# indygreg/python-zstandard

Measured on AMD Instinct MI355X. Metric: GB/s uncompressed throughput, batch decompress of 128 KiB level-3 frames (the decompress half of BASELINE.json's metric; the compress half on the same inputs is this line's 'compress' object), higher is better.
Workload: dtype u8

## Files before the change

python-zstandard_amd/csrc/zhip_decode_kernel.hpp:

```cpp
#pragma once
#include "zhip_device.hpp"
#include "zhip_format.hpp"
#include "zhip_xxh64.hpp"

#if defined(ZHIP_EMU) && defined(ZD_TRACE)
#include <stdio.h>
extern "C" { extern long zd_trace_pos; extern long zd_cur_frame; extern long zd_stat[16]; }
#define ZD_STAT(i, v) do { if (zh_lane() == 0) zd_stat[i] += (v); } while (0)
#define ZD_TRR(lo, n, what, a1, a2) do { if (zh_lane() == 0 && zd_trace_pos + 40 >= (long)(lo) && zd_trace_pos < (long)(lo) + (long)(n) + 40) fprintf(stderr, "[trace] f%ld range [%ld,+%ld) %s %ld %ld\n", zd_cur_frame, (long)(lo), (long)(n), what, (long)(a1), (long)(a2)); } while (0)
#define ZD_TR(pos, what, a1, a2, a3) do { if ((long)(pos) == zd_trace_pos) fprintf(stderr, "[trace] f%ld pos=%ld %s lane=%u %ld %ld %ld\n", zd_cur_frame, (long)(pos), what, zh_lane(), (long)(a1), (long)(a2), (long)(a3)); } while (0)
#else
#define ZD_TR(pos, what, a1, a2, a3) do { } while (0)
#define ZD_TRR(lo, n, what, a1, a2) do { } while (0)
#define ZD_STAT(i, v) do { } while (0)
#endif
#define ZD_STAGE_BYTES 512
#define ZD_ASM_BYTES 4096
#define ZD_COOP_LEN 32

ZH_CONST uint32_t zc_llBase[36] = {0,1,2,3,4,5,6,7,8,9,10,11,12,13,14,15,16,18,20,22,24,28,32,40,48,64,128,256,512,
                                   1024,2048,4096,8192,16384,32768,65536};
ZH_CONST uint8_t zc_llBits[36] = {0,0,0,0,0,0,0,0,0,0,0,0,0,0,0,0,1,1,1,1,2,2,3,3,4,6,7,8,9,10,11,12,13,14,15,16};
ZH_CONST uint32_t zc_mlBase[53] = {3,4,5,6,7,8,9,10,11,12,13,14,15,16,17,18,19,20,21,22,23,24,25,26,27,28,29,30,31,32,
                                   33,34,35,37,39,41,43,47,51,59,67,83,99,131,259,515,1027,2051,4099,8195,16387,32771,65539};
// ... 417 lines not shown
    }
    zh_sync();
    return (int)log;
}

ZH_DEVFN bool zd_huf_stream(const uint16_t* huf, uint32_t log, const uint8_t* src, uint32_t srcSize, uint8_t* out, uint32_t count)
{
    ZdPBits b;
    if (!zd_pb_init(b, src, srcSize)) return false;
    uint32_t i = 0;
    zd_pb_norm(b);
    while (i + 4 <= count) {
        uint32_t e0 = huf[zd_pb_peek(b, log)]; b.used += e0 >> 8;
        uint32_t e1 = huf[zd_pb_peek(b, log)]; b.used += e1 >> 8;
        uint32_t e2 = huf[zd_pb_peek(b, log)]; b.used += e2 >> 8;
        uint32_t e3 = huf[zd_pb_peek(b, log)]; b.used += e3 >> 8;
        if (b.used > 64) return false;
        zh_st32(out + i, (e0 & 255) | ((e1 & 255) << 8) | ((e2 & 255) << 16) | ((e3 & 255) << 24));
        i += 4;
        zd_pb_norm(b);
    }
    while (i < count) {
        uint32_t e = huf[zd_pb_peek(b, log)]; b.used += e >> 8;
        if (b.used > 64) return false;
        out[i++] = (uint8_t)e;
    }
    zd_pb_norm(b);
    return zd_pb_done(b);
}

struct ZdLitDefer { uint16_t* table; uint32_t maxLog; uint32_t taken, log, four, streamBytes; const uint8_t* streams;
                    const uint16_t* prevTable; uint32_t prevLog;
                    uint32_t shared, shareOK;
                    const ZpPre* pre; };
ZH_DEVFN int zd_literals(ZdLDS& L, ZdState& st, const uint8_t* src, uint32_t srcSize, uint8_t* lit, uint32_t blockMax, ZdProf& P,
                         ZdLitDefer* defer = nullptr)
{
    const uint32_t lane = zh_lane();
    if (srcSize < 1) return -ZE_CORRUPTION;
    uint32_t b0 = src[0], type = b0 & 3, fmt = (b0 >> 2) & 3;
    uint32_t hdr, regen, csize = 0, four = 0;
    st.litRLE = 0;
    if (type < 2) {
        if (fmt == 1) { if (srcSize < 2) return -ZE_CORRUPTION; hdr = 2; regen = zh_ld16(src) >> 4; }
        else if (fmt == 3) { if (srcSize < 3) return -ZE_CORRUPTION; hdr = 3; regen = zh_ld24(src) >> 4; }
        else { hdr = 1; regen = b0 >> 3; }
        if (regen > blockMax) return -ZE_CORRUPTION;
        st.litSize = regen;
        if (type == 0) {
            if (hdr + regen > srcSize) return -ZE_CORRUPTION;
            st.litPtr = src + hdr;
            return (int)(hdr + regen);
        }
        if (hdr + 1 > srcSize) return -ZE_CORRUPTION;
        st.litRLE = 1; st.rleByte = src[hdr]; st.litPtr = lit;
        return (int)(hdr + 1);
    }
    if (srcSize < 5) return -ZE_CORRUPTION;
    uint32_t v = zh_ld32(src);
    if (fmt < 2) { hdr = 3; four = fmt; regen = (v >> 4) & 0x3FF; csize = (v >> 14) & 0x3FF; }
    else if (fmt == 2) { hdr = 4; four = 1; regen = (v >> 4) & 0x3FFF; csize = v >> 18; }
    else { hdr = 5; four = 1; regen = (v >> 4) & 0x3FFFF; csize = (v >> 22) + ((uint32_t)src[4] << 10); }
    if (regen > blockMax || regen > ZF_BLOCK_MAX) return -ZE_CORRUPTION;
    if (!four && regen == 0) return -ZE_CORRUPTION;
    if (four && regen < 6) return -ZE_CORRUPTION;
    if (hdr + csize > srcSize) return -ZE_CORRUPTION;
    const uint8_t* p = src + hdr; uint32_t left = csize;
    if (type == 3) {
        if (st.hufCount == 0) return -ZE_DICT_CORRUPTED;
    } else {
        uint32_t cnt = 0, lg = 0;
        int r = zd_read_huf_weights(L, p, left, &cnt, &lg, defer ? defer->pre : nullptr, hdr);
        if (r < 0) return -ZE_CORRUPTION;
        p += r; left -= (uint32_t)r; st.hufCount = cnt;
    }
    if (type == 3 && defer && defer->prevTable) {
        const int lgp = (int)defer->prevLog;
        if (four) {
            if (left < 10) return -ZE_CORRUPTION;
            if (3 * ((regen + 3) / 4) > regen) return -ZE_CORRUPTION;
        }
        if (defer->shareOK) defer->shared = 1;
        else {
            const uint64_t* t8 = (const uint64_t*)defer->prevTable; uint64_t* g8 = (uint64_t*)defer->table;
            for (uint32_t i = lane; i < (1u << lgp) / 4 + ((1u << lgp) < 4 ? 1u : 0u); i += 64) g8[i] = t8[i];
        }
        defer->taken = 1; defer->log = (uint32_t)lgp; defer->four = four; defer->streamBytes = left; defer->streams = p;
        ZD_T(P, ZP_HUFTAB);
        st.litPtr = lit; st.litSize = regen;
        return (int)(hdr + csize);
    }
    int lg = zd_build_huf(L, st.hufCount);
    if (lg < 0) return -ZE_CORRUPTION;
    if (defer && (uint32_t)lg <= defer->maxLog) {
        if (four) {
// ... 594 lines not shown
```

python-zstandard_amd/csrc/zhip_decode_pipeline.hpp:

```cpp
#pragma once
#include "zhip_decode_kernel.hpp"

ZH_DEV void zp_pack_fse(ZdLDS& L, uint32_t* T, uint32_t llLog, uint32_t ofLog, uint32_t mlLog)
{
    const uint32_t lane = zh_lane();
    for (uint32_t u = lane; u < ZP_FSE_CELLS / 2; u += 64) {
        const uint32_t lg = u < 256 ? llLog : u < 512 ? mlLog : ofLog;
        const uint32_t local = (2 * u) & (u < 512 ? 511u : 255u);
        uint32_t pair = 0;
        for (uint32_t k = 0; k < 2; k++) {
            uint32_t cell = 0;
            if (local + k < (1u << lg)) {
                const uint32_t e = L.fse[2 * u + k];
                cell = ((e >> 19) << 10) | (((e & 1023) + (1u << lg)) >> ((e >> 10) & 15));
            }
            pair |= cell << (16 * k);
        }
        T[u] = pair;
    }
}

struct ZpHdr { uint32_t pos, blockMax, hasChecksum, skippable; uint64_t fcs; };
ZH_DEV int zp_frame_header(const ZhipPipeArgs& a, const uint8_t* src, uint32_t srcSize, ZpHdr& h)
{
    const uint32_t mg = a.magicless ? 0u : 4u;
    h.skippable = 0;
    if (srcSize < mg + 1) return ZE_SRC_SIZE_WRONG;
    if (mg && (zh_ld32(src) & 0xFFFFFFF0u) == ZF_MAGIC_SKIPPABLE) {
        if (srcSize < 8 || (uint64_t)zh_ld32(src + 4) + 8 > srcSize) return ZE_SRC_SIZE_WRONG;
        h.skippable = 1; h.pos = 0; h.blockMax = 0; h.hasChecksum = 0; h.fcs = 0;
        return 0;
    }
    if (mg && zh_ld32(src) != ZF_MAGIC) return ZE_PREFIX_UNKNOWN;
    const uint32_t fhd = src[mg];
    const uint32_t dictCode = fhd & 3, single = (fhd >> 5) & 1, fcsCode = fhd >> 6;
    h.hasChecksum = (fhd >> 2) & 1;
    const uint32_t dictBytes = dictCode == 3 ? 4 : dictCode;
    const uint32_t fcsBytes = fcsCode == 0 ? single : (1u << fcsCode);
    const uint32_t hs = mg + 1 + (single ? 0 : 1) + dictBytes + fcsBytes;
    if (fhd & 8) return ZE_FRAMEPARAM_UNSUPPORTED;
    if (srcSize < hs) return ZE_SRC_SIZE_WRONG;
    uint32_t pos = mg + 1;
    uint64_t windowSize = 0;
    if (!single) {
        const uint32_t wd = src[pos++], wl = 10 + (wd >> 3);
        if (wl > 31) return ZE_WINDOW_TOO_LARGE;
        windowSize = 1ull << wl; windowSize += (windowSize >> 3) * (wd & 7);
    }
    {   const uint32_t dictID = dictCode == 0 ? 0u : dictCode == 1 ? src[pos] : dictCode == 2 ? zh_ld16(src + pos) : zh_ld32(src + pos);
        pos += dictBytes;
        if (dictID && dictID != a.dictID) return ZE_DICT_WRONG; }
    uint64_t fcs = ~0ull;
    if (fcsCode == 0) { if (single) fcs = src[pos]; }
    else if (fcsCode == 1) fcs = (uint64_t)zh_ld16(src + pos) + 256;
    else if (fcsCode == 2) fcs = zh_ld32(src + pos);
    else fcs = zh_ld64(src + pos);
    pos += fcsBytes;
    if (single) windowSize = fcs;
    if (windowSize > a.maxWindowSize) return ZE_WINDOW_TOO_LARGE;
    h.blockMax = windowSize < ZF_BLOCK_MAX ? (uint32_t)windowSize : ZF_BLOCK_MAX;
    h.fcs = fcs; h.pos = pos;
    return 0;
}

ZH_DEVFN int zp_block_tables(const ZhipPipeArgs& a, ZdLDS& L, ZdState& st, ZdLitDefer& df, const uint8_t* src, uint32_t pos, uint32_t bs,
                             uint32_t blockMax, uint32_t t, ZdMeta& m, ZdProf& P, bool share, bool dictInLds)
{
    const uint32_t lane = zh_lane();
    uint8_t* lit;
    {
        uint32_t need16 = 0;
        if (bs >= 5 && (src[pos] & 3u) >= 2u) {
            const uint32_t v = zh_ld32(src + pos), fmt = (v >> 2) & 3u;
            const uint32_t regen = fmt < 2 ? (v >> 4) & 0x3FFu : fmt == 2 ? (v >> 4) & 0x3FFFu : (v >> 4) & 0x3FFFFu;
            if (regen <= ZF_BLOCK_MAX) need16 = (regen + 256u + 15u) >> 4;
        }
        uint32_t lb = 0;
        if (need16) {
            lb = zh_first(zh_atomic_add(a.counters + 8, lane == 0 ? need16 : 0u));
            if ((uint64_t)lb + need16 > a.arenaBudget16) {
                if (zh_opaque(lane) == 0) zh_atomic_add(a.counters + 8, 0u - need16);
                return ZP_RC_FALLBACK;
            }
        }
        const uint32_t lpos = need16 ? a.arenaBudget16 - lb - need16 : 0u;
        lit = a.litArena + (size_t)lpos * 16;
        if (zh_opaque(lane) == 0) a.bases[2 * (size_t)t + 1] = lpos;
    }
    st.litPtr = lit; st.litSize = 0; st.litRLE = 0; st.rleByte = 0;
    const ZhipDictEntropy* const de = a.dictEntropy;
    const int r = zd_literals(L, st, src + pos, bs, lit, blockMax, P, &df);
    if (r < 0) return -r;
    m.litSize = st.litSize;
    if (df.taken) { m.litMode = 3u | (df.log << 8) | (df.four << 16) | (df.shared ? ZP_LIT_SHARED : 0u); m.litOff = (uint32_t)(df.streams - src); m.produced = df.streamBytes; }
    else if (st.litRLE) { m.litMode = 2; m.litOff = st.rleByte; }
    else if (st.litPtr == lit) { m.litMode = 1; m.litOff = 0; }
    else { m.litMode = 0; m.litOff = (uint32_t)(st.litPtr - src); }
    const uint8_t* sp = src + pos + (uint32_t)r; const uint8_t* const send = src + pos + bs;
    if (sp >= send) return ZE_SRC_SIZE_WRONG;
    uint32_t nbSeq = *sp++;
    if (nbSeq > 127) {
        if (nbSeq == 255) { if (sp + 2 > send) return ZE_SRC_SIZE_WRONG; nbSeq = zh_ld16(sp) + 0x7F00; sp += 2; }
        else { if (sp >= send) return ZE_SRC_SIZE_WRONG; nbSeq = ((nbSeq - 128) << 8) + *sp++; }
    }
    m.nbSeq = nbSeq;
    if (nbSeq == 0) { if (sp != send) return ZE_CORRUPTION; }
    else {
        if (nbSeq > ZP_SEQ_CAP - 16) return ZE_CORRUPTION;
        if (sp >= send) return ZE_SRC_SIZE_WRONG;
        const uint32_t modes = *sp++;
        if (modes & 3) return ZE_CORRUPTION;
        const bool allShared = share && de && (modes >> 2) == 0x3F;
        if (allShared) {
            st.llLog = de->llLog; st.ofLog = de->ofLog; st.mlLog = de->mlLog;
            if (sp >= send) return ZE_CORRUPTION;
        } else {
            if (de && !dictInLds) {
                zh_sync();
                const uint32_t* T = a.dictTables->fse;
                if ((modes >> 6) == 3) { for (uint32_t k = lane; k < (1u << de->llLog); k += 64) L.fse[ZD_FSE_LL + k] = T[ZD_FSE_LL + k]; st.llLog = de->llLog; }
                if (((modes >> 4) & 3) == 3) { for (uint32_t k = lane; k < (1u << de->ofLog); k += 64) L.fse[ZD_FSE_OF + k] = T[ZD_FSE_OF + k]; st.ofLog = de->ofLog; }
                if (((modes >> 2) & 3) == 3) { for (uint32_t k = lane; k < (1u << de->mlLog); k += 64) L.fse[ZD_FSE_ML + k] = T[ZD_FSE_ML + k]; st.mlLog = de->mlLog; }
                zh_sync();
            }
            const uint32_t hn = (uint32_t)(send - sp) < 256u ? (uint32_t)(send - sp) : 256u;
            uint8_t* const stg = (uint8_t*)L.u.huf + 4096;
            zh_sync();
            zd_stage_wave(stg, sp, hn);
            zh_sync();
            const uint8_t* lp = stg; const uint8_t* const lend = stg + hn;
            const ZpPre* const spre = df.pre && df.pre->seqAt == (uint32_t)(sp - (src + pos)) ? df.pre : nullptr;
            int q = zd_seq_table(L, modes >> 6, ZD_KIND_LL, &st.llLog, lp, lend, spre); if (q < 0) return -q; sp += q; lp += q;
            q = zd_seq_table(L, (modes >> 4) & 3, ZD_KIND_OF, &st.ofLog, lp, lend, spre); if (q < 0) return -q; sp += q; lp += q;
            q = zd_seq_table(L, (modes >> 2) & 3, ZD_KIND_ML, &st.mlLog, lp, lend, spre); if (q < 0) return -q; sp += q; lp += q;
            if (sp >= send) return ZE_CORRUPTION;
            zh_sync();
            uint32_t* const T = (uint32_t*)(a.fseTables + (size_t)t * ZP_FSE_CELLS);
            zp_pack_fse(L, T, st.llLog, st.ofLog, st.mlLog);
        }
        m.logs = st.llLog | (st.ofLog << 8) | (st.mlLog << 16) | (allShared ? ZP_LOGS_SHARED : 0u);
    }
    m.seqOff = (uint32_t)(sp - src); m.seqEnd = pos + bs;
    ZD_T(P, ZP_SEQTAB);
    return 0;
}

ZH_DEV void zp_enter_bins(const ZhipPipeArgs& a, ZdMeta& m)
{
    const uint32_t ks = m.nbSeq ? 1u + (m.nbSeq >> ZP_BIN_SHIFT) : 0u;
    const uint32_t kl = (m.litMode & 255u) == 3u ? 1u + (m.litSize >> ZP_LITBIN_SHIFT) : 0u;
    if (ks) m.pad = zh_atomic_add(a.counters + ZP_CNT_BINS + (256 - (ks > 256 ? 256u : ks)), 1u);
    if (kl) m.hasChecksum |= zh_atomic_add(a.counters + ZP_CNT_BINS + 256 + (256 - (kl > 256 ? 256u : kl)), 1u) << 1;
}
ZH_DEV void zp_enter_bins_wave(const ZhipPipeArgs& a, ZdMeta& m, bool on)
{
    const uint32_t lane = zh_lane();
    const uint32_t ks = on && m.nbSeq ? 1u + (m.nbSeq >> ZP_BIN_SHIFT) : 0u;
    const uint32_t kl = on && (m.litMode & 255u) == 3u ? 1u + (m.litSize >> ZP_LITBIN_SHIFT) : 0u;
    const uint32_t bS = ks ? 256u - (ks > 256u ? 256u : ks) : 0xFFFFu, bL = kl ? 256u + (256u - (kl > 256u ? 256u : kl)) : 0xFFFFu;
#pragma unroll
    for (int which = 0; which < 2; which++) {
        const uint32_t mine = which ? bL : bS;
        uint64_t todo = zh_ballot(mine != 0xFFFFu);
        while (todo) {
            const uint32_t leader = (uint32_t)zh_ctz64(todo);
            const uint32_t b = zh_shfl(mine, leader);
            const uint64_t same = zh_ballot(mine == b);
            uint32_t base = 0;
            if (lane == leader) base = zh_atomic_add(a.counters + ZP_CNT_BINS + b, (uint32_t)zh_popc64(same));
            base = zh_shfl(base, leader);
            if (mine == b) { const uint32_t rank = base + (uint32_t)zh_popc64(same & zh_lt_mask()); if (which) m.hasChecksum |= rank << 1; else m.pad = rank; }
            todo &= ~same;
        }
    }
}
ZH_DEV void zp_meta_clear(ZdMeta& m)
{
    m.status = 0; m.path = 0; m.seqOff = m.seqEnd = 0; m.litSize = 0; m.litMode = 0; m.litOff = 0; m.nbSeq = 0;
    m.blockMax = 0; m.fcsLo = m.fcsHi = 0xFFFFFFFFu; m.produced = 0; m.hasChecksum = 0; m.checksum = 0; m.logs = 0; m.pad = 0;
}

ZH_DEV bool zp_lit_shared_try(const ZhipPipeArgs& a, uint32_t f, ZdMeta& m, uint32_t& need16)
{
    zp_meta_clear(m); need16 = 0;
    if (!a.dictEntropy->hufCount || a.dictTables->hufLog > ZP_HUF_LOGMAX) return false;
// ... 134 lines not shown
    }
    for (uint32_t u = 0; u < size; u++) {
        const uint32_t q = S.symAt[u], x = S.next[q];
        S.next[q] = (uint8_t)(x + 1);
        const uint32_t nb = tl - (uint32_t)zh_highbit32(x);
        S.cell[u] = (uint16_t)(((x << nb) - size) | (nb << 6) | (q << 9));
    }
    ZdBits b; uint32_t cnt = 0;
    if (!zd_bits_init(b, desc + r, hb - (uint32_t)r)) return;
    zd_bits_reload(b);
    uint32_t s1 = zd_bits_peek(b, tl); b.used += tl;
    uint32_t s2 = zd_bits_peek(b, tl); b.used += tl;
    if (tl == 0) { s1 = s2 = 0; }
    int64_t left;
    for (;;) {
        if (b.used >= 32) zd_bits_reload(b);
        left = (int64_t)(b.ptr - b.start) * 8 + 64 - (int64_t)b.used;
        const uint32_t e1 = S.cell[s1], nb1 = (e1 >> 6) & 7;
        if (cnt > 253) return;
        R.weights[cnt++] = (uint8_t)(e1 >> 9);
        const uint32_t v1 = nb1 ? zd_bits_peek(b, nb1) : 0; b.used += nb1; left -= nb1;
        s1 = (e1 & 63) + v1;
        const uint32_t e2 = S.cell[s2], nb2 = (e2 >> 6) & 7;
        if (left < 0) { R.weights[cnt++] = (uint8_t)(e2 >> 9); break; }
        if (cnt > 253) return;
        R.weights[cnt++] = (uint8_t)(e2 >> 9);
        const uint32_t v2 = nb2 ? zd_bits_peek(b, nb2) : 0; b.used += nb2; left -= nb2;
        s2 = (e2 & 63) + v2;
        if (left < 0) { R.weights[cnt++] = (uint8_t)(S.cell[s1] >> 9); break; }
    }
    R.wAt = at; R.wCount = cnt;
}

ZH_DEV void zp_pre_one(const ZhipPipeArgs& a, uint32_t f, ZpPre& R, ZpPreLane& S)
{
    R.wCount = 0; R.wAt = 0; R.seqAt = 0; R.t[0].valid = 0; R.t[1].valid = 0; R.t[2].valid = 0;
    const uint8_t* src = a.src + a.srcSegs[2 * (size_t)f];
    const uint64_t srcSize64 = a.srcSegs[2 * (size_t)f + 1];
    if (srcSize64 > 0x7FFFFFFFull) return;
    const uint32_t srcSize = (uint32_t)srcSize64;
    ZpHdr h;
    if (zp_frame_header(a, src, srcSize, h) || h.skippable) return;
    uint32_t pos = h.pos;
    if (pos + 3 > srcSize) return;
    const uint32_t bh = zh_ld24(src + pos); pos += 3;
    const uint32_t bs = bh >> 3;
    if (!(bh & 1) || ((bh >> 1) & 3) != 2) return;
    if (pos + bs > srcSize || bs > h.blockMax || bs < 2) return;
    const uint8_t* const b = src + pos;
    const uint32_t b0 = b[0], lt = b0 & 3, fmt = (b0 >> 2) & 3;
    uint32_t used, regen;
    if (lt < 2) {
        uint32_t hdr;
        if (fmt == 1) { hdr = 2; regen = zh_ld16(b) >> 4; }
        else if (fmt == 3) { if (bs < 3) return; hdr = 3; regen = zh_ld24(b) >> 4; }
        else { hdr = 1; regen = b0 >> 3; }
        if (regen > h.blockMax) return;
        if (lt == 0) { if (hdr + regen > bs) return; used = hdr + regen; }
        else { if (hdr + 1 > bs) return; used = hdr + 1; }
    } else {
        if (bs < 5) return;
        const uint32_t v = zh_ld32(b);
        uint32_t hdr, four, csize;
        if (fmt < 2) { hdr = 3; four = fmt; regen = (v >> 4) & 0x3FF; csize = (v >> 14) & 0x3FF; }
        else if (fmt == 2) { hdr = 4; four = 1; regen = (v >> 4) & 0x3FFF; csize = v >> 18; }
        else { hdr = 5; four = 1; regen = (v >> 4) & 0x3FFFF; csize = (v >> 22) + ((uint32_t)b[4] << 10); }
        if (regen > h.blockMax || regen > ZF_BLOCK_MAX) return;
        if (four ? regen < 6 : regen == 0) return;
        if (hdr + csize > bs) return;
        used = hdr + csize;
        if (lt == 2 && csize >= 1) {
            const uint32_t hb = b[hdr];
            if (hb >= 2 && hb < 128 && 1 + hb <= csize) zp_pre_weights(R, S, b + hdr + 1, hb, hdr);
        }
    }
    uint32_t sp = used; const uint32_t send = bs;
    if (sp >= send) return;
    uint32_t nbSeq = b[sp++];
    if (nbSeq > 127) {
        if (nbSeq == 255) { if (sp + 2 > send) return; nbSeq = zh_ld16(b + sp) + 0x7F00; sp += 2; }
        else { if (sp >= send) return; nbSeq = ((nbSeq - 128) << 8) + b[sp++]; }
    }
    if (nbSeq == 0 || nbSeq > ZP_SEQ_CAP - 16 || sp >= send) return;
    const uint32_t modes = b[sp++];
    if (modes & 3) return;
    const uint32_t hn = send - sp < 256u ? send - sp : 256u;
    const uint8_t* lp = b + sp; const uint8_t* const lend = lp + hn;
    R.seqAt = sp;
#pragma unroll
    for (int kind = 0; kind < 3; kind++) {
        const uint32_t mode = kind == ZD_KIND_LL ? modes >> 6 : kind == ZD_KIND_OF ? (modes >> 4) & 3 : (modes >> 2) & 3;
        if (mode == 3) return;
        if (mode == 1) { if (lp >= lend) return; lp += 1; }
        if (mode == 2) {
            uint32_t ms = kind == ZD_KIND_LL ? ZF_MAXLL : kind == ZD_KIND_ML ? ZF_MAXML : ZF_MAXOFF, tl = 0;
            const int r = zd_read_ncount_to(R.norm[kind], lp, lend, &ms, &tl);
            if (r < 0) return;
            R.t[kind].maxSym = ms; R.t[kind].log = tl; R.t[kind].used = (uint32_t)r; R.t[kind].valid = 1;
            lp += r;
        }
    }
}

ZH_DEVFN void zp_pre_body(const ZhipPipeArgs& a, ZpPreLDS& L)
{
    const uint32_t lane = zh_lane();
    for (;;) {
        const uint32_t base = zh_first(zh_atomic_add(a.counters + 11, lane == 0 ? 64u : 0u));
        if (base >= a.count) break;
        const uint32_t i = base + lane;
        if (i < a.count) zp_pre_one(a, a.first + i, a.pre[i], L.lane[lane]);
    }
}

ZH_DEVFN void zp_lit_body(const ZhipPipeArgs& a, ZdLDS& L)
{
    const uint32_t lane = zh_lane();
    if (lane < 36) { L.llBase[lane] = zc_llBase[lane]; L.llBits[lane] = zc_llBits[lane]; }
    if (lane < 53) { L.mlBase[lane] = zc_mlBase[lane]; L.mlBits[lane] = zc_mlBits[lane]; }
    zh_sync();
    bool anyCk = false;
    for (;;) {
        const uint32_t got = zh_atomic_add(a.counters + 0, lane == 0 ? 1u : 0u);
        if (zh_opaque(lane) == 0) L.misc[7] = got;
        zh_sync();
        const uint32_t got1 = zh_first(L.misc[7]);
        zh_sync();
        if (got1 >= (a.k1Lanes ? a.counters[10] : a.count)) { if (anyCk && zh_opaque(lane) == 0) *(volatile uint32_t*)(a.counters + 12) = 1u; break; }
        const uint32_t i = a.k1Lanes ? a.order[got1] : got1;
        const uint32_t f = a.first + i;
        ZdMeta m;
        zp_meta_clear(m);
        const uint8_t* src = a.src + a.srcSegs[2 * (size_t)f];
        const uint64_t srcSize64 = a.srcSegs[2 * (size_t)f + 1];
        uint8_t* dst = a.dst + a.dstSegs[2 * (size_t)f];
        const uint64_t cap64 = a.dstSegs[2 * (size_t)f + 1];
        int err = 0; bool fallback = false;
        ZdProf P; P.on = a.prof != nullptr;
        if (P.on) { for (int q = 0; q < ZP_N; q++) P.acc[q] = 0; P.t0 = zd_clock(); }
        do {
            if (srcSize64 > 0x7FFFFFFFull) { fallback = true; break; }
            const uint32_t srcSize = (uint32_t)srcSize64;
            const uint32_t cap = cap64 > 0x7FFFFFFFull ? 0x7FFFFFFFu : (uint32_t)cap64;
            ZpHdr h;
            err = zp_frame_header(a, src, srcSize, h);
            if (err || h.skippable) break;
            const uint32_t blockMax = h.blockMax, hasChecksum = h.hasChecksum;
            const uint64_t fcs = h.fcs;
            uint32_t pos = h.pos;
            m.blockMax = blockMax; m.fcsLo = (uint32_t)fcs; m.fcsHi = (uint32_t)(fcs >> 32);
            if (pos + 3 > srcSize) { err = ZE_SRC_SIZE_WRONG; break; }
            const uint32_t bh = zh_ld24(src + pos); pos += 3;
            const uint32_t lastBlock = bh & 1, type = (bh >> 1) & 3, bs = bh >> 3;
            if (!lastBlock) { fallback = true; break; }
            if (type == 3) { err = ZE_CORRUPTION; break; }
            const bool onePass = fcs != ~0ull && cap64 >= fcs;
            if (type < 2) {
                if (type == 0 ? pos + bs > srcSize : pos + 1 > srcSize) { err = ZE_SRC_SIZE_WRONG; break; }
                if (bs > blockMax && !onePass) { err = ZE_CORRUPTION; break; }
                if (bs > cap) { err = ZE_DST_TOO_SMALL; break; }
                if (type == 0) zd_copy_wave(dst, src + pos, bs); else zd_fill_wave(dst, src[pos], bs);
                if (fcs != ~0ull && fcs != bs) { err = ZE_CORRUPTION; break; }
                m.produced = bs;
                if (hasChecksum && a.ckLater) {
                    const uint32_t cpos = pos + (type == 0 ? bs : 1);
                    if (cpos + 4 > srcSize) { err = ZE_CHECKSUM_WRONG; break; }
                    m.hasChecksum = 1; m.checksum = zh_ld32(src + cpos);
                    anyCk = true;
                } else if (hasChecksum) {
                    const uint32_t cpos = pos + (type == 0 ? bs : 1);
                    if (cpos + 4 > srcSize) { err = ZE_CHECKSUM_WRONG; break; }
                    zd_fence();
                    zh_sync();
                    if (zh_opaque(lane) == 0) L.misc[0] = (uint32_t)ze_xxh64(dst, bs);
                    zh_sync();
                    const uint32_t digest = zh_first(L.misc[0]);
                    zh_sync();
                    if (digest != zh_ld32(src + cpos)) { err = ZE_CHECKSUM_WRONG; break; }
                }
                break;
            }
            if (pos + bs > srcSize) { err = ZE_SRC_SIZE_WRONG; break; }
            if (bs > blockMax) { err = onePass ? ZE_SRC_SIZE_WRONG : ZE_CORRUPTION; break; }
            if (bs < 2) { err = ZE_CORRUPTION; break; }
            ZdState st;
            st.rep0 = 1; st.rep1 = 4; st.rep2 = 8; st.hufCount = 0; st.llLog = st.ofLog = st.mlLog = 0xFF;
            ZD_T(P, ZP_HEADER);
            ZdLitDefer df; df.table = a.hufTables + (size_t)i * ZP_HUF_CELLS; df.maxLog = ZP_HUF_LOGMAX; df.taken = 0;
            df.log = 0; df.four = 0; df.streamBytes = 0; df.streams = src; df.prevTable = nullptr; df.prevLog = 0; df.shared = 0; df.shareOK = 1;
            df.pre = a.pre ? a.pre + i : nullptr;
            const ZhipDictEntropy* const de = a.dictEntropy;
            if (de) {
                st.hufCount = de->hufCount;
                if (a.dictTables->hufLog <= ZP_HUF_LOGMAX) { df.prevTable = a.dictTables->huf; df.prevLog = a.dictTables->hufLog; }
                else { zh_sync(); for (uint32_t k = lane; k < 256; k += 64) L.weights[k] = de->hufWeights[k]; zh_sync(); }
            }
            err = zp_block_tables(a, L, st, df, src, pos, bs, blockMax, i, m, P, true, false);
            if (err == (int)ZP_RC_FALLBACK) { err = 0; fallback = true; break; }
            if (err) break;
            if (hasChecksum) {
                if (pos + bs + 4 > srcSize) { err = ZE_CHECKSUM_WRONG; break; }
                m.hasChecksum = 1; m.checksum = zh_ld32(src + pos + bs);
                anyCk = anyCk || a.ckLater != 0;
            }
            m.path = 1;
        } while (false);
        if (fallback) { m.path = 2; }
        if (err) { m.status = err; m.path = 0; }
        zh_sync();
        if (zh_opaque(lane) == 0) {
            if (m.path == 1) zp_enter_bins(a, m);
            a.meta[i] = m;
            if (m.path == 2) { const uint32_t k = zh_atomic_add(a.fallbackCount, 1u); a.fallbackList[k] = f; }
            if (m.path == 0) { a.status[f] = m.status; a.outSizes[f] = m.status ? 0 : m.produced; }
        }
#ifdef ZHIP_EMU
        zd_fence();
#endif
        if (P.on) { ZD_T(P, ZP_RAW); if (lane == 0) for (int q = 0; q < ZP_N; q++) if (P.acc[q]) zh_atomic_add64(a.prof + q, P.acc[q]); }
    }
}

ZH_DEVFN void zp_lit_mb_body(const ZhipPipeArgs& a, ZdLDS& L)
{
    const uint32_t lane = zh_lane();
    if (lane < 36) { L.llBase[lane] = zc_llBase[lane]; L.llBits[lane] = zc_llBits[lane]; }
    if (lane < 53) { L.mlBase[lane] = zc_mlBase[lane]; L.mlBits[lane] = zc_mlBits[lane]; }
    zh_sync();
    bool anyCk = false;
    for (;;) {
        const uint32_t got = zh_atomic_add(a.counters + 0, lane == 0 ? 1u : 0u);
        if (zh_opaque(lane) == 0) L.misc[7] = got;
        zh_sync();
        const uint32_t i = zh_first(L.misc[7]);
        zh_sync();
        if (i >= a.count) { if (anyCk && zh_opaque(lane) == 0) *(volatile uint32_t*)(a.counters + 12) = 1u; break; }
        const uint32_t f = a.first + i;
        const uint8_t* src = a.src + a.srcSegs[2 * (size_t)f];
        const uint64_t srcSize64 = a.srcSegs[2 * (size_t)f + 1];
        const uint64_t cap64 = a.dstSegs[2 * (size_t)f + 1];
        ZpFrameRec rec; rec.firstItem = 0; rec.nItems = 0; rec.path = 0; rec.blockMax = 0; rec.fcsLo = rec.fcsHi = 0xFFFFFFFFu; rec.hasChecksum = 0; rec.checksum = 0;
        int err = 0; bool fallback = false;
        ZdProf P; P.on = false;
        do {
            if (srcSize64 > 0x7FFFFFFFull) { fallback = true; break; }
            const uint32_t srcSize = (uint32_t)srcSize64;
            ZpHdr h;
            err = zp_frame_header(a, src, srcSize, h);
            if (err || h.skippable) break;
            const uint32_t blockMax = h.blockMax;
            const uint64_t fcs = h.fcs;
            rec.blockMax = blockMax; rec.fcsLo = (uint32_t)fcs; rec.fcsHi = (uint32_t)(fcs >> 32);
            const bool onePass = fcs != ~0ull && cap64 >= fcs;
            uint32_t nb = 0, end = h.pos;
            for (;;) {
// ... 19 lines not shown
                ZdMeta z; zp_meta_clear(z);
                for (uint32_t t = base + lane; t < a.itemCap && t - base < nb; t += 64) { a.meta[t] = z; a.itemFrame[t] = i; }
                fallback = true; break;
            }
            rec.firstItem = base; rec.nItems = nb;
            ZdState st;
            st.rep0 = 1; st.rep1 = 4; st.rep2 = 8; st.hufCount = 0; st.llLog = st.ofLog = st.mlLog = 0xFF;
            const uint16_t* prevTable = nullptr; uint32_t prevLog = 0;
            const ZhipDictEntropy* const de = a.dictEntropy;
            if (de) {
                st.hufCount = de->hufCount;
                if (a.dictTables->hufLog <= ZP_HUF_LOGMAX) { prevTable = a.dictTables->huf; prevLog = a.dictTables->hufLog; }
                zh_sync();
                for (uint32_t k = lane; k < 256; k += 64) L.weights[k] = de->hufWeights[k];
                const uint32_t* T = a.dictTables->fse;
                for (uint32_t k = lane; k < 1280; k += 64) L.fse[k] = T[k];
                st.llLog = de->llLog; st.ofLog = de->ofLog; st.mlLog = de->mlLog;
                zh_sync();
            }
            uint32_t pos = h.pos;
            for (uint32_t j = 0; j < nb; j++) {
                const uint32_t t = base + j;
                ZdMeta m; zp_meta_clear(m);
                const uint32_t bh = zh_ld24(src + pos); pos += 3;
                const uint32_t type = (bh >> 1) & 3, bs = bh >> 3;
                if (err || fallback) {  }
                else if (type < 2) {
                    if (bs > blockMax && !onePass) err = ZE_CORRUPTION;
                    else { m.path = type == 0 ? 3u : 4u; m.litSize = bs; m.litOff = type == 0 ? pos : (uint32_t)src[pos]; }
                } else if (bs > blockMax) err = onePass ? ZE_SRC_SIZE_WRONG : ZE_CORRUPTION;
                else if (bs < 2) err = ZE_CORRUPTION;
                else {
                    ZdLitDefer df; df.table = a.hufTables + (size_t)t * ZP_HUF_CELLS; df.maxLog = ZP_HUF_LOGMAX; df.taken = 0;
                    df.log = 0; df.four = 0; df.streamBytes = 0; df.streams = src; df.prevTable = prevTable; df.prevLog = prevLog; df.shared = 0; df.shareOK = 0; df.pre = nullptr;
                    err = zp_block_tables(a, L, st, df, src, pos, bs, blockMax, t, m, P, false, true);
                    if (err == (int)ZP_RC_FALLBACK) { err = 0; fallback = true; }
                    else if (!err) {
                        m.path = 1;
                        const uint32_t lt = src[pos] & 3;
                        if (lt >= 2) {
                            if (df.taken) { prevTable = df.table; prevLog = df.log; } else { prevTable = nullptr; prevLog = 0; }
                        }
                    }
                }
                if (err && m.status == 0) { m.status = err; m.path = 0; }
                pos += type == 1 ? 1u : bs;
                zh_sync();
                if (zh_opaque(lane) == 0) {
                    if (m.path == 1) zp_enter_bins(a, m);
                    a.meta[t] = m; a.itemFrame[t] = i;
                }
                zh_sync();
            }
            err = 0;
            if (fallback) break;
            rec.path = 1;
        } while (false);
        if (fallback) rec.path = 2;
        if (err) rec.path = 0;
        zh_sync();
        if (zh_opaque(lane) == 0) {
            a.frameRecs[i] = rec;
            if (rec.path == 2) { const uint32_t k = zh_atomic_add(a.fallbackCount, 1u); a.fallbackList[k] = f; }
            if (rec.path == 0) { a.status[f] = err; a.outSizes[f] = 0; }
        }
#ifdef ZHIP_EMU
        zd_fence();
#endif
// ... 850 lines not shown
```

python-zstandard_amd/csrc/zhip_format.hpp:

```cpp
#pragma once
#include <stdint.h>

enum {
    ZE_OK = 0, ZE_GENERIC = 1, ZE_PREFIX_UNKNOWN = 10, ZE_FRAMEPARAM_UNSUPPORTED = 14, ZE_WINDOW_TOO_LARGE = 16,
    ZE_CORRUPTION = 20, ZE_CHECKSUM_WRONG = 22, ZE_LITERALS_HEADER_WRONG = 24, ZE_DICT_CORRUPTED = 30,
    ZE_DICT_WRONG = 32, ZE_PARAM_UNSUPPORTED = 40, ZE_PARAM_OUTOFBOUND = 42, ZE_TABLELOG_TOO_LARGE = 44, ZE_MAXSYMBOL_TOO_LARGE = 46,
    ZE_MAXSYMBOL_TOO_SMALL = 48, ZE_MEMORY = 64, ZE_DST_TOO_SMALL = 70, ZE_SRC_SIZE_WRONG = 72
};

#define ZF_MAGIC 0xFD2FB528u
#define ZF_MAGIC_SKIPPABLE 0x184D2A50u
#define ZF_DICT_MAGIC 0xEC30A437u
#define ZF_BLOCK_MAX (1u << 17)
#define ZF_MAXLL 35
#define ZF_MAXML 52
#define ZF_MAXOFF 31
#define ZF_LL_LOGMAX 9
#define ZF_ML_LOGMAX 9
#define ZF_OF_LOGMAX 8

#define ZHIP_LIT_STRIDE (ZF_BLOCK_MAX + 256)

struct ZhipDictEntropy {
    uint8_t  hufWeights[256];
// ... 163 lines not shown
#define ZP_FSE_CELLS 1280
#define ZP_K2_STRIDE 2564
#define ZP_HUF_LOGMAX 11
#define ZP_HUF_CELLS (1u << ZP_HUF_LOGMAX)
#ifndef ZP_HUF_FRAMES
#define ZP_HUF_FRAMES 12
#endif
#define ZP_HUF_LS (ZP_HUF_FRAMES > 8 ? 6 : ZP_HUF_FRAMES > 4 ? 5 : 4)
#define ZP_LITBIN_SHIFT 9
#define ZP_BIN_SHIFT 7

#define ZP_CNT_BINS 16u
#define ZP_CNT_WORDS (16u + 512u)

struct ZpFrameRec {
    uint32_t firstItem, nItems;
    uint32_t path;
    uint32_t blockMax;
    uint32_t fcsLo, fcsHi;
    uint32_t hasChecksum, checksum;
};
#define ZP_OF_LIMIT 0x1E000000u
#define ZP_SYM_REP(k) (0x1E800000u + ((uint32_t)(k) << 23))
#define ZP_SYM_TOP ZP_SYM_REP(2)
#define ZP_MB_MAXBLOCKS 4096u
#define ZP_RC_FALLBACK 0x7FFF0002
struct alignas(16) ZpPre {
    uint8_t weights[256];
    int16_t norm[3][64];
    uint32_t wCount;
    uint32_t wAt;
    struct { uint32_t valid, maxSym, log, used; } t[3];
    uint32_t seqAt;
    uint32_t pad;
};
struct ZhipPipeArgs {
    const uint8_t* src; const uint64_t* srcSegs;
    uint8_t* dst; const uint64_t* dstSegs;
    uint64_t* outSizes; int32_t* status;
    ZdMeta* meta;
    uint8_t* litArena;
    uint64_t* seqArena;
    uint32_t* bases;
    uint32_t arenaBudget16;
    uint16_t* fseTables;
    uint32_t* order;
    uint16_t* hufTables;
    uint32_t* orderLit;
    uint32_t* counters;
    uint32_t* fallbackCount;
    uint32_t* fallbackList;
    uint32_t first, count;
    uint32_t itemCap;
    uint32_t* itemFrame;
    uint32_t* itemReps;
    ZpFrameRec* frameRecs;
    uint64_t maxWindowSize;
    uint32_t magicless;
    uint32_t ckLater;
    ZpPre* pre;
    uint32_t k1Lanes;
    unsigned long long* prof;
    uint32_t dictID, dictContentSize;
    const uint8_t* dictContent;
    const ZhipDictEntropy* dictEntropy;
    const ZhipDictTables* dictTables;
};
// ... 1 lines not shown
```

Measured before the change: 394.9.

## Claim work ahead, stage headers in LDS, pre-claim literal arena in K0

In the per-frame literal/table kernel, the next work-item claim is issued one iteration ahead so its atomic latency overlaps the current frame. Frame and literal header bytes are staged once into LDS, and the sequence header is staged early so scattered global loads are avoided. The pre-pass kernel now reserves literal arena space with one wave-wide scan and atomic per 64 frames instead of a per-frame atomic in K1. Bin-rank writes to meta are deferred to the next iteration to hide atomic latency. These add extra syncs, extra LDS use and more complex state, and the arena budget may be over-reserved.

```diff
diff --git a/python-zstandard_amd/csrc/zhip_decode_kernel.hpp b/python-zstandard_amd/csrc/zhip_decode_kernel.hpp
--- a/python-zstandard_amd/csrc/zhip_decode_kernel.hpp
+++ b/python-zstandard_amd/csrc/zhip_decode_kernel.hpp
@@ -473,18 +473,21 @@
 struct ZdLitDefer { uint16_t* table; uint32_t maxLog; uint32_t taken, log, four, streamBytes; const uint8_t* streams;
                     const uint16_t* prevTable; uint32_t prevLog;
                     uint32_t shared, shareOK;
-                    const ZpPre* pre; };
+                    const ZpPre* pre;
+                    uint64_t hdr8; uint32_t hdrOK; };
 ZH_DEVFN int zd_literals(ZdLDS& L, ZdState& st, const uint8_t* src, uint32_t srcSize, uint8_t* lit, uint32_t blockMax, ZdProf& P,
                          ZdLitDefer* defer = nullptr)
 {
     const uint32_t lane = zh_lane();
     if (srcSize < 1) return -ZE_CORRUPTION;
-    uint32_t b0 = src[0], type = b0 & 3, fmt = (b0 >> 2) & 3;
+    const bool hv = defer && defer->hdrOK;
+    const uint64_t h8 = hv ? defer->hdr8 : 0;
+    uint32_t b0 = hv ? (uint32_t)h8 & 255u : (uint32_t)src[0], type = b0 & 3, fmt = (b0 >> 2) & 3;
     uint32_t hdr, regen, csize = 0, four = 0;
     st.litRLE = 0;
     if (type < 2) {
-        if (fmt == 1) { if (srcSize < 2) return -ZE_CORRUPTION; hdr = 2; regen = zh_ld16(src) >> 4; }
-        else if (fmt == 3) { if (srcSize < 3) return -ZE_CORRUPTION; hdr = 3; regen = zh_ld24(src) >> 4; }
+        if (fmt == 1) { if (srcSize < 2) return -ZE_CORRUPTION; hdr = 2; regen = (hv ? (uint32_t)h8 & 0xFFFFu : zh_ld16(src)) >> 4; }
+        else if (fmt == 3) { if (srcSize < 3) return -ZE_CORRUPTION; hdr = 3; regen = (hv ? (uint32_t)h8 & 0xFFFFFFu : zh_ld24(src)) >> 4; }
         else { hdr = 1; regen = b0 >> 3; }
         if (regen > blockMax) return -ZE_CORRUPTION;
         st.litSize = regen;
@@ -498,10 +501,10 @@
         return (int)(hdr + 1);
     }
     if (srcSize < 5) return -ZE_CORRUPTION;
-    uint32_t v = zh_ld32(src);
+    uint32_t v = hv ? (uint32_t)h8 : zh_ld32(src);
     if (fmt < 2) { hdr = 3; four = fmt; regen = (v >> 4) & 0x3FF; csize = (v >> 14) & 0x3FF; }
     else if (fmt == 2) { hdr = 4; four = 1; regen = (v >> 4) & 0x3FFF; csize = v >> 18; }
-    else { hdr = 5; four = 1; regen = (v >> 4) & 0x3FFFF; csize = (v >> 22) + ((uint32_t)src[4] << 10); }
+    else { hdr = 5; four = 1; regen = (v >> 4) & 0x3FFFF; csize = (v >> 22) + ((hv ? (uint32_t)(h8 >> 32) & 255u : (uint32_t)src[4]) << 10); }
     if (regen > blockMax || regen > ZF_BLOCK_MAX) return -ZE_CORRUPTION;
     if (!four && regen == 0) return -ZE_CORRUPTION;
     if (four && regen < 6) return -ZE_CORRUPTION;
diff --git a/python-zstandard_amd/csrc/zhip_decode_pipeline.hpp b/python-zstandard_amd/csrc/zhip_decode_pipeline.hpp
--- a/python-zstandard_amd/csrc/zhip_decode_pipeline.hpp
+++ b/python-zstandard_amd/csrc/zhip_decode_pipeline.hpp
@@ -1,5 +1,19 @@
 #pragma once
 #include "zhip_decode_kernel.hpp"
+
+#ifndef ZP_K1_HDR_COPY
+#define ZP_K1_HDR_COPY 1
+#endif
+#ifndef ZP_K1_CLAIM_AHEAD
+#define ZP_K1_CLAIM_AHEAD 1
+#endif
+#ifndef ZP_K0_LIT_CLAIM
+#define ZP_K0_LIT_CLAIM 1
+#endif
+#ifndef ZP_K1_BINS_LATE
+#define ZP_K1_BINS_LATE 1
+#endif
+#define ZP_HDR_AT (4096u + 1024u)
 
 ZH_DEV void zp_pack_fse(ZdLDS& L, uint32_t* T, uint32_t llLog, uint32_t ofLog, uint32_t mlLog)
 {
@@ -63,20 +77,27 @@
     return 0;
 }
 
+struct ZpK1Held { uint64_t lit8; uint32_t lit8OK, room16, roomBase; };
 ZH_DEVFN int zp_block_tables(const ZhipPipeArgs& a, ZdLDS& L, ZdState& st, ZdLitDefer& df, const uint8_t* src, uint32_t pos, uint32_t bs,
-                             uint32_t blockMax, uint32_t t, ZdMeta& m, ZdProf& P, bool share, bool dictInLds)
+                             uint32_t blockMax, uint32_t t, ZdMeta& m, ZdProf& P, bool share, bool dictInLds, const ZpK1Held kh)
 {
     const uint32_t lane = zh_lane();
     uint8_t* lit;
     {
         uint32_t need16 = 0;
-        if (bs >= 5 && (src[pos] & 3u) >= 2u) {
-            const uint32_t v = zh_ld32(src + pos), fmt = (v >> 2) & 3u;
+        if (bs >= 5 && ((kh.lit8OK ? (uint32_t)kh.lit8 : (uint32_t)src[pos]) & 3u) >= 2u) {
+            const uint32_t v = kh.lit8OK ? (uint32_t)kh.lit8 : zh_ld32(src + pos), fmt = (v >> 2) & 3u;
             const uint32_t regen = fmt < 2 ? (v >> 4) & 0x3FFu : fmt == 2 ? (v >> 4) & 0x3FFFu : (v >> 4) & 0x3FFFFu;
             if (regen <= ZF_BLOCK_MAX) need16 = (regen + 256u + 15u) >> 4;
         }
         uint32_t lb = 0;
-        if (need16) {
+        const bool roomHeld = ZP_K0_LIT_CLAIM && need16 && kh.room16 == need16;
+        if (roomHeld) {
+            lb = kh.roomBase;
+#ifdef ZHIP_EMU
+            if (lane == 0) zd_stat[12]++;
+#endif
+        } else if (need16) {
             lb = zh_first(zh_atomic_add(a.counters + 8, lane == 0 ? need16 : 0u));
             if ((uint64_t)lb + need16 > a.arenaBudget16) {
                 if (zh_opaque(lane) == 0) zh_atomic_add(a.counters + 8, 0u - need16);
@@ -89,6 +110,7 @@
     }
     st.litPtr = lit; st.litSize = 0; st.litRLE = 0; st.rleByte = 0;
     const ZhipDictEntropy* const de = a.dictEntropy;
+    df.hdr8 = kh.lit8; df.hdrOK = kh.lit8OK;
     const int r = zd_literals(L, st, src + pos, bs, lit, blockMax, P, &df);
     if (r < 0) return -r;
     m.litSize = st.litSize;
@@ -98,17 +120,27 @@
     else { m.litMode = 0; m.litOff = (uint32_t)(st.litPtr - src); }
     const uint8_t* sp = src + pos + (uint32_t)r; const uint8_t* const send = src + pos + bs;
     if (sp >= send) return ZE_SRC_SIZE_WRONG;
-    uint32_t nbSeq = *sp++;
+    uint8_t* const stg = (uint8_t*)L.u.huf + 4096;
+#if ZP_K1_HDR_COPY
+    {   const uint32_t sn = (uint32_t)(send - sp) < 260u ? (uint32_t)(send - sp) : 260u;
+        zh_sync();
+        zd_stage_wave(stg, sp, sn);
+        zh_sync(); }
+    const uint8_t* cp = stg;
+#else
+    const uint8_t* cp = sp;
+#endif
+    uint32_t nbSeq = *cp++; sp++;
     if (nbSeq > 127) {
-        if (nbSeq == 255) { if (sp + 2 > send) return ZE_SRC_SIZE_WRONG; nbSeq = zh_ld16(sp) + 0x7F00; sp += 2; }
-        else { if (sp >= send) return ZE_SRC_SIZE_WRONG; nbSeq = ((nbSeq - 128) << 8) + *sp++; }
+        if (nbSeq == 255) { if (sp + 2 > send) return ZE_SRC_SIZE_WRONG; nbSeq = zh_ld16(cp) + 0x7F00; sp += 2; cp += 2; }
+        else { if (sp >= send) return ZE_SRC_SIZE_WRONG; nbSeq = ((nbSeq - 128) << 8) + *cp++; sp++; }
     }
     m.nbSeq = nbSeq;
     if (nbSeq == 0) { if (sp != send) return ZE_CORRUPTION; }
     else {
         if (nbSeq > ZP_SEQ_CAP - 16) return ZE_CORRUPTION;
         if (sp >= send) return ZE_SRC_SIZE_WRONG;
-        const uint32_t modes = *sp++;
+        const uint32_t modes = *cp++; sp++;
         if (modes & 3) return ZE_CORRUPTION;
         const bool allShared = share && de && (modes >> 2) == 0x3F;
         if (allShared) {
@@ -124,11 +156,14 @@
                 zh_sync();
             }
             const uint32_t hn = (uint32_t)(send - sp) < 256u ? (uint32_t)(send - sp) : 256u;
-            uint8_t* const stg = (uint8_t*)L.u.huf + 4096;
+#if ZP_K1_HDR_COPY
+            const uint8_t* lp = cp; const uint8_t* const lend = lp + hn;
+#else
             zh_sync();
             zd_stage_wave(stg, sp, hn);
             zh_sync();
             const uint8_t* lp = stg; const uint8_t* const lend = stg + hn;
+#endif
             const ZpPre* const spre = df.pre && df.pre->seqAt == (uint32_t)(sp - (src + pos)) ? df.pre : nullptr;
             int q = zd_seq_table(L, modes >> 6, ZD_KIND_LL, &st.llLog, lp, lend, spre); if (q < 0) return -q; sp += q; lp += q;
             q = zd_seq_table(L, (modes >> 4) & 3, ZD_KIND_OF, &st.ofLog, lp, lend, spre); if (q < 0) return -q; sp += q; lp += q;
@@ -151,6 +186,19 @@
     const uint32_t kl = (m.litMode & 255u) == 3u ? 1u + (m.litSize >> ZP_LITBIN_SHIFT) : 0u;
     if (ks) m.pad = zh_atomic_add(a.counters + ZP_CNT_BINS + (256 - (ks > 256 ? 256u : ks)), 1u);
     if (kl) m.hasChecksum |= zh_atomic_add(a.counters + ZP_CNT_BINS + 256 + (256 - (kl > 256 ? 256u : kl)), 1u) << 1;
+}
+ZH_DEV uint32_t zp_enter_bins_issue(const ZhipPipeArgs& a, const ZdMeta& m, uint32_t& rs, uint32_t& rl)
+{
+    const uint32_t ks = m.nbSeq ? 1u + (m.nbSeq >> ZP_BIN_SHIFT) : 0u;
+    const uint32_t kl = (m.litMode & 255u) == 3u ? 1u + (m.litSize >> ZP_LITBIN_SHIFT) : 0u;
+    if (ks) rs = zh_atomic_add(a.counters + ZP_CNT_BINS + (256 - (ks > 256 ? 256u : ks)), 1u);
+    if (kl) rl = zh_atomic_add(a.counters + ZP_CNT_BINS + 256 + (256 - (kl > 256 ? 256u : kl)), 1u);
+    return (ks ? 1u : 0u) | (kl ? 2u : 0u);
+}
+ZH_DEV void zp_late_ranks(const ZhipPipeArgs& a, uint32_t i, uint32_t how, uint32_t rs, uint32_t rl, uint32_t hc)
+{
+    if (how & 1u) a.meta[i].pad = rs;
+    if (how & 2u) a.meta[i].hasChecksum = hc | (rl << 1);
 }
 ZH_DEV void zp_enter_bins_wave(const ZhipPipeArgs& a, ZdMeta& m, bool on)
 {
@@ -351,9 +399,9 @@
     R.wAt = at; R.wCount = cnt;
 }
 
-ZH_DEV void zp_pre_one(const ZhipPipeArgs& a, uint32_t f, ZpPre& R, ZpPreLane& S)
-{
-    R.wCount = 0; R.wAt = 0; R.seqAt = 0; R.t[0].valid = 0; R.t[1].valid = 0; R.t[2].valid = 0;
+ZH_DEV void zp_pre_one(const ZhipPipeArgs& a, uint32_t f, ZpPre& R, ZpPreLane& S, uint32_t& need16)
+{
+    R.wCount = 0; R.wAt = 0; R.seqAt = 0; R.t[0].valid = 0; R.t[1].valid = 0; R.t[2].valid = 0; R.lit16 = 0; R.litBase = 0;
     const uint8_t* src = a.src + a.srcSegs[2 * (size_t)f];
     const uint64_t srcSize64 = a.srcSegs[2 * (size_t)f + 1];
     if (srcSize64 > 0x7FFFFFFFull) return;
@@ -388,6 +436,7 @@
         if (four ? regen < 6 : regen == 0) return;
         if (hdr + csize > bs) return;
         used = hdr + csize;
+        need16 = (regen + 256u + 15u) >> 4;
         if (lt == 2 && csize >= 1) {
             const uint32_t hb = b[hdr];
             if (hb >= 2 && hb < 128 && 1 + hb <= csize) zp_pre_weights(R, S, b + hdr + 1, hb, hdr);
@@ -428,25 +477,67 @@
         const uint32_t base = zh_first(zh_atomic_add(a.counters + 11, lane == 0 ? 64u : 0u));
         if (base >= a.count) break;
         const uint32_t i = base + lane;
-        if (i < a.count) zp_pre_one(a, a.first + i, a.pre[i], L.lane[lane]);
-    }
-}
-
+        uint32_t need16 = 0;
+        if (i < a.count) zp_pre_one(a, a.first + i, a.pre[i], L.lane[lane], need16);
+#if ZP_K0_LIT_CLAIM
+        const uint32_t incl = zh_scan_add(need16), total = zh_shfl(incl, 63);
+        if (total) {
+            const uint32_t lb = zh_first(zh_atomic_add(a.counters + 8, lane == 0 ? total : 0u));
+            if ((uint64_t)lb + total > a.arenaBudget16) {
+                if (zh_opaque(lane) == 0) {
+                    zh_atomic_add(a.counters + 8, 0u - total);
+#ifdef ZHIP_EMU
+                    zd_stat[14]++;
+#endif
+                }
+            } else if (need16) {
+                a.pre[i].lit16 = need16; a.pre[i].litBase = lb + incl - need16;
+#ifdef ZHIP_EMU
+                zd_stat[13]++;
+#endif
+            }
+        }
+#endif
+    }
+}
+
+ZH_DEV uint32_t zp_claim_issue(const ZhipPipeArgs& a)
+{
+    uint32_t v = zh_opaque(0u);
+    if (zh_opaque(zh_lane()) == 0) v = zh_atomic_add(a.counters + zh_opaque(0u), 1u);
+    return v;
+}
 ZH_DEVFN void zp_lit_body(const ZhipPipeArgs& a, ZdLDS& L)
 {
     const uint32_t lane = zh_lane();
+    const uint32_t bound = a.k1Lanes ? a.counters[10] : a.count;
     if (lane < 36) { L.llBase[lane] = zc_llBase[lane]; L.llBits[lane] = zc_llBits[lane]; }
     if (lane < 53) { L.mlBase[lane] = zc_mlBase[lane]; L.mlBits[lane] = zc_mlBits[lane]; }
     zh_sync();
     bool anyCk = false;
+#if ZP_K1_CLAIM_AHEAD
+    uint32_t claimed = zh_first(zp_claim_issue(a)), claimedI = zh_first(a.k1Lanes && claimed < bound ? a.order[claimed] : claimed);
+#endif
+#if ZP_K1_BINS_LATE
+    uint32_t lateHow = 0, lateI = 0, lateS = 0, lateL = 0, lateHc = 0;
+#endif
     for (;;) {
+#if ZP_K1_CLAIM_AHEAD
+        const uint32_t got1 = claimed;
+#else
         const uint32_t got = zh_atomic_add(a.counters + 0, lane == 0 ? 1u : 0u);
         if (zh_opaque(lane) == 0) L.misc[7] = got;
         zh_sync();
         const uint32_t got1 = zh_first(L.misc[7]);
         zh_sync();
-        if (got1 >= (a.k1Lanes ? a.counters[10] : a.count)) { if (anyCk && zh_opaque(lane) == 0) *(volatile uint32_t*)(a.counters + 12) = 1u; break; }
+#endif
+        if (got1 >= bound) { if (anyCk && zh_opaque(lane) == 0) *(volatile uint32_t*)(a.counters + 12) = 1u; break; }
+#if ZP_K1_CLAIM_AHEAD
+        const uint32_t ahead = zp_claim_issue(a);
+        const uint32_t i = claimedI;
+#else
         const uint32_t i = a.k1Lanes ? a.order[got1] : got1;
+#endif
         const uint32_t f = a.first + i;
         ZdMeta m;
         zp_meta_clear(m);
@@ -454,6 +545,24 @@
         const uint64_t srcSize64 = a.srcSegs[2 * (size_t)f + 1];
         uint8_t* dst = a.dst + a.dstSegs[2 * (size_t)f];
         const uint64_t cap64 = a.dstSegs[2 * (size_t)f + 1];
+        ZpK1Held kh; kh.lit8 = 0; kh.lit8OK = 0; kh.room16 = 0; kh.roomBase = 0;
+#if ZP_K0_LIT_CLAIM
+        if (a.pre) { kh.room16 = a.pre[i].lit16; kh.roomBase = a.pre[i].litBase; }
+#endif
+#if ZP_K1_HDR_COPY
+        uint8_t* const hp = (uint8_t*)L.u.huf + ZP_HDR_AT;
+        if (lane < (srcSize64 < 64u ? (uint32_t)srcSize64 : 64u)) hp[lane] = src[lane];
+        zh_sync();
+#else
+        const uint8_t* const hp = src;
+#endif
+#if ZP_K1_CLAIM_AHEAD
+        claimed = zh_first(ahead); claimedI = zh_first(a.k1Lanes && claimed < bound ? a.order[claimed] : claimed);
+#endif
+#if ZP_K1_BINS_LATE
+        if (zh_opaque(lane) == 0 && lateHow) zp_late_ranks(a, lateI, lateHow, lateS, lateL, lateHc);
+        lateHow = 0;
+#endif
         int err = 0; bool fallback = false;
         ZdProf P; P.on = a.prof != nullptr;
         if (P.on) { for (int q = 0; q < ZP_N; q++) P.acc[q] = 0; P.t0 = zd_clock(); }
@@ -462,14 +571,14 @@
             const uint32_t srcSize = (uint32_t)srcSize64;
             const uint32_t cap = cap64 > 0x7FFFFFFFull ? 0x7FFFFFFFu : (uint32_t)cap64;
             ZpHdr h;
-            err = zp_frame_header(a, src, srcSize, h);
+            err = zp_frame_header(a, hp, srcSize, h);
             if (err || h.skippable) break;
             const uint32_t blockMax = h.blockMax, hasChecksum = h.hasChecksum;
             const uint64_t fcs = h.fcs;
             uint32_t pos = h.pos;
             m.blockMax = blockMax; m.fcsLo = (uint32_t)fcs; m.fcsHi = (uint32_t)(fcs >> 32);
             if (pos + 3 > srcSize) { err = ZE_SRC_SIZE_WRONG; break; }
-            const uint32_t bh = zh_ld24(src + pos); pos += 3;
+            const uint32_t bh = zh_ld24(hp + pos); pos += 3;
             const uint32_t lastBlock = bh & 1, type = (bh >> 1) & 3, bs = bh >> 3;
             if (!lastBlock) { fallback = true; break; }
             if (type == 3) { err = ZE_CORRUPTION; break; }
@@ -478,7 +587,7 @@
                 if (type == 0 ? pos + bs > srcSize : pos + 1 > srcSize) { err = ZE_SRC_SIZE_WRONG; break; }
                 if (bs > blockMax && !onePass) { err = ZE_CORRUPTION; break; }
                 if (bs > cap) { err = ZE_DST_TOO_SMALL; break; }
-                if (type == 0) zd_copy_wave(dst, src + pos, bs); else zd_fill_wave(dst, src[pos], bs);
+                if (type == 0) zd_copy_wave(dst, src + pos, bs); else zd_fill_wave(dst, hp[pos], bs);
                 if (fcs != ~0ull && fcs != bs) { err = ZE_CORRUPTION; break; }
                 m.produced = bs;
                 if (hasChecksum && a.ckLater) {
@@ -508,13 +617,16 @@
             ZdLitDefer df; df.table = a.hufTables + (size_t)i * ZP_HUF_CELLS; df.maxLog = ZP_HUF_LOGMAX; df.taken = 0;
             df.log = 0; df.four = 0; df.streamBytes = 0; df.streams = src; df.prevTable = nullptr; df.prevLog = 0; df.shared = 0; df.shareOK = 1;
             df.pre = a.pre ? a.pre + i : nullptr;
+#if ZP_K1_HDR_COPY
+            kh.lit8 = (uint64_t)zh_ld32(hp + pos) | ((uint64_t)zh_ld32(hp + pos + 4) << 32); kh.lit8OK = 1;
+#endif
             const ZhipDictEntropy* const de = a.dictEntropy;
             if (de) {
                 st.hufCount = de->hufCount;
                 if (a.dictTables->hufLog <= ZP_HUF_LOGMAX) { df.prevTable = a.dictTables->huf; df.prevLog = a.dictTables->hufLog; }
                 else { zh_sync(); for (uint32_t k = lane; k < 256; k += 64) L.weights[k] = de->hufWeights[k]; zh_sync(); }
             }
-            err = zp_block_tables(a, L, st, df, src, pos, bs, blockMax, i, m, P, true, false);
+            err = zp_block_tables(a, L, st, df, src, pos, bs, blockMax, i, m, P, true, false, kh);
             if (err == (int)ZP_RC_FALLBACK) { err = 0; fallback = true; break; }
             if (err) break;
             if (hasChecksum) {
@@ -528,7 +640,11 @@
         if (err) { m.status = err; m.path = 0; }
         zh_sync();
         if (zh_opaque(lane) == 0) {
+#if ZP_K1_BINS_LATE
+            if (m.path == 1) { lateHow = zp_enter_bins_issue(a, m, lateS, lateL); lateI = i; lateHc = m.hasChecksum; }
+#else
             if (m.path == 1) zp_enter_bins(a, m);
+#endif
             a.meta[i] = m;
             if (m.path == 2) { const uint32_t k = zh_atomic_add(a.fallbackCount, 1u); a.fallbackList[k] = f; }
             if (m.path == 0) { a.status[f] = m.status; a.outSizes[f] = m.status ? 0 : m.produced; }
@@ -538,8 +654,10 @@
 #endif
         if (P.on) { ZD_T(P, ZP_RAW); if (lane == 0) for (int q = 0; q < ZP_N; q++) if (P.acc[q]) zh_atomic_add64(a.prof + q, P.acc[q]); }
     }
-}
-
+#if ZP_K1_BINS_LATE
+    if (zh_opaque(lane) == 0 && lateHow) zp_late_ranks(a, lateI, lateHow, lateS, lateL, lateHc);
+#endif
+}
 ZH_DEVFN void zp_lit_mb_body(const ZhipPipeArgs& a, ZdLDS& L)
 {
     const uint32_t lane = zh_lane();
@@ -625,8 +743,9 @@
                 else if (bs < 2) err = ZE_CORRUPTION;
                 else {
                     ZdLitDefer df; df.table = a.hufTables + (size_t)t * ZP_HUF_CELLS; df.maxLog = ZP_HUF_LOGMAX; df.taken = 0;
-                    df.log = 0; df.four = 0; df.streamBytes = 0; df.streams = src; df.prevTable = prevTable; df.prevLog = prevLog; df.shared = 0; df.shareOK = 0; df.pre = nullptr;
-                    err = zp_block_tables(a, L, st, df, src, pos, bs, blockMax, t, m, P, false, true);
+                    df.log = 0; df.four = 0; df.streamBytes = 0; df.streams = src; df.prevTable = prevTable; df.prevLog = prevLog; df.shared = 0; df.shareOK = 0; df.pre = nullptr; df.hdr8 = 0; df.hdrOK = 0;
+                    ZpK1Held kh; kh.lit8 = 0; kh.lit8OK = 0; kh.room16 = 0; kh.roomBase = 0;
+                    err = zp_block_tables(a, L, st, df, src, pos, bs, blockMax, t, m, P, false, true, kh);
                     if (err == (int)ZP_RC_FALLBACK) { err = 0; fallback = true; }
                     else if (!err) {
                         m.path = 1;
diff --git a/python-zstandard_amd/csrc/zhip_format.hpp b/python-zstandard_amd/csrc/zhip_format.hpp
--- a/python-zstandard_amd/csrc/zhip_format.hpp
+++ b/python-zstandard_amd/csrc/zhip_format.hpp
@@ -219,7 +219,9 @@
     uint32_t wAt;
     struct { uint32_t valid, maxSym, log, used; } t[3];
     uint32_t seqAt;
-    uint32_t pad;
+    uint32_t lit16;
+    uint32_t litBase;
+    uint32_t pad[3];
 };
 struct ZhipPipeArgs {
     const uint8_t* src; const uint64_t* srcSegs;
```

Result: no change. 396.9 (median of 6 runs) (+0.5%).
